# lbcb-sci/raven

Measured on AMD Instinct MI355X. Metric: read Gbase/s through overlap+polish, higher is better.
Workload: dtype u32

## Files before the change

### raven_amd/csrc/engine.h

```cpp
#pragma once

#include <atomic>
#include <memory>
#include <mutex>
#include <string>
#include <vector>

#include "common.h"

namespace rvn {

constexpr int kSketchTile = 1024;
constexpr int kMaxWindow = 256;

inline u64 next_reads_serial() {
  static std::atomic<u64> counter{0};
  return ++counter;
}

struct ReadsDev {
  u32 n = 0;
  u64 total_bases = 0;
  u64 n_words = 0;
  DevBuf packed;
// ... 23 lines not shown
};

struct Index {
  u64 m = 0;
  u64 u = 0;
  int table_bits = 0;
  int shift = 0;
  DevBuf s_val[2];
  DevBuf s_org[2];
  int cur = 0;
  DevBuf u_val;
  DevBuf u_start;
  DevBuf table;
  DevBuf direct;
  bool direct_built = false;
  u32 occurrence = 0xFFFFFFFFu;
  bool table_built = false;
  bool has_query_flags = false;
  bool all_query = false;
  u32 first = 0, last = 0;
};

struct MapOut {
  u32 first = 0, last = 0;
  u64 n_query = 0;
  u64 n_matches = 0;
  u64 n_intervals = 0;
  u64 n_overlaps = 0;
  DevBuf ovl;
  DevBuf ovl_read_off;
// ... 8 lines not shown
  enum { kSketch, kSort, kIndex, kFilter, kQuery, kMatch, kSegSort, kIntervals, kChain, kCompact, kMerge, kPile,
         kTruncate, kNum };
  double ms[kNum] = {};
  u64 launches[kNum] = {};
};

struct PileState;
struct PileRegion;
struct ResolveState;

struct EngineOptions {
  long long nw_budget_mb = 0;
  long long nw_group_walk = 0;
  long long nw_stripe_lanes = 0;
  long long index_direct_min_keys = 0;
  long long poa_rows_min_windows = -1;
  long long io_threads = 0;
  long long io_slab_mb = 0;
  long long io_ring = 0;
  long long io_zlib = 0;
  long long arena_mb = 0;
  long long arena_margin_mb = 0;
  long long no_arena = 0;
  long long release_always = 0;
  long long polish_join = 0;
  long long polish_sketch_cache_mb = -1;
};
const char* engine_option_names();
long long* engine_option(EngineOptions& o, const char* name);

// ... 15 lines not shown
  u64 shard_join_matches = 0;
  MapOut map_out;
  DevBuf tmp_a, tmp_b, tmp_c, tmp_d, tmp_e, tmp_f, scan_tmp, sort_tmp;
  DevBuf sh_hist, sh_off, sh_ptrs;
  DevBuf q_start, q_cnt, m_off;
  struct PolishSketch {
    u32 first = 0, last = 0;
    Sketch sk;
  };
  u64 polish_sketch_owner = 0;
  std::vector<std::unique_ptr<PolishSketch>> polish_sketches;
  DevBuf pl_tval, pl_torg;
  DevBuf foreign_val, foreign_org;
  DevBuf sketch_sum;
  DevBuf m_grp[2], m_pos[2];
  DevBuf seg_off, iv_slot_begin, iv_slot_end, iv_cnt, iv_off, iv_begin, iv_end;
  DevBuf lis_min, lis_pred, lis_tail, lis_mask, ovl_slots, ovl_flags, ovl_scan, chain_big;
  DevBuf poa_scratch, poa2_scratch, polish_quals;
  DevBuf ed_cnt, ed_sort, ed_todo;
  DevBuf p2_slot, p2_pairs, p2_dist, p2_regions, p2_index_of, p2_kmers_off, p2_ok, p2_keep, p2_tmp_ovl;
  DevBuf io_text[2];
  int stage_kind = 0;
  u32 oom_mask = 0;
  std::vector<std::pair<std::unique_ptr<PinBuf>, bool>> io_pin;
  DevBuf poa_sched, poa_redo_w, poa_redo_i;
  DevBuf nw_hs, nw_ck, nw_hs2, nw_ck2, nw_hs3, nw_ck3, nw_hs4, nw_ck4, nw_strip, nw_jobs, nw_res;
  double nw_rate = -1.0;
  DevBuf pl_best, pl_best_t, pl_idmap, pl_recs, pl_keep, pl_win_cnt, pl_win_off, pl_win_fill, pl_win_meta, pl_first_window,
      pl_keys, pl_lays_tmp, pl_lays, pl_wins, pl_out, pl_len, pl_status, pl_ok, pl_cons_off, pl_final, pl_qual_off, pl_misc;
  std::vector<u64> pl_last_off;
// ... 302 lines not shown
```

### raven_amd/csrc/engine.hip

```cpp
#include <chrono>
#include <memory>

#include "abi.h"
#include "poa.h"

using namespace rvn;

static_assert(sizeof(rvn_overlap) == sizeof(rvn::Overlap), "overlap layout");

namespace {

thread_local std::string g_err;

const char* kStageNames[StageTimes::kNum] = {"sketch", "sort", "index", "filter", "query_sketch", "match",
                                             "seg_sort", "intervals", "chain", "compact", "merge", "pile",
                                             "truncate"};

void swap_bufs(DevBuf& a, DevBuf& b) {
  std::swap(a.ptr, b.ptr);
  std::swap(a.cap, b.cap);
}

}

// ... 62 lines not shown
  }
}

void fetch_values(Engine& e, const DevBuf& val, u64 n, u64* values) {
  if (!values || n == 0) return;
  if (e.val64) {
    RVN_HIP(hipMemcpy(values, val.ptr, n * 8, hipMemcpyDeviceToHost));
  } else {
    std::vector<u32> tmp(n);
    RVN_HIP(hipMemcpy(tmp.data(), val.ptr, n * 4, hipMemcpyDeviceToHost));
    for (u64 i = 0; i < n; ++i) values[i] = tmp[i];
  }
}

const char* engine_option_names() {
  return "nw_budget_mb, nw_group_walk, nw_stripe_lanes, index_direct_min_keys, poa_rows_min_windows, io_threads, io_slab_mb, io_ring, io_zlib, arena_mb, arena_margin_mb, "
         "no_arena, release_always, polish_join, polish_sketch_cache_mb";
}
long long* engine_option(EngineOptions& o, const char* name) {
  const std::string n(name ? name : "");
  if (n == "nw_budget_mb") return &o.nw_budget_mb;
  if (n == "nw_group_walk") return &o.nw_group_walk;
  if (n == "nw_stripe_lanes") return &o.nw_stripe_lanes;
  if (n == "index_direct_min_keys") return &o.index_direct_min_keys;
  if (n == "poa_rows_min_windows") return &o.poa_rows_min_windows;
  if (n == "io_threads") return &o.io_threads;
  if (n == "io_slab_mb") return &o.io_slab_mb;
  if (n == "io_ring") return &o.io_ring;
  if (n == "io_zlib") return &o.io_zlib;
  if (n == "arena_mb") return &o.arena_mb;
  if (n == "arena_margin_mb") return &o.arena_margin_mb;
  if (n == "no_arena") return &o.no_arena;
  if (n == "release_always") return &o.release_always;
  if (n == "polish_join") return &o.polish_join;
  if (n == "polish_sketch_cache_mb") return &o.polish_sketch_cache_mb;
  return nullptr;
}

void engine_release_scratch(Engine& e) {
  if (e.stream) (void)rvn_stream_sync(e.stream);
  e.query_ready = false;
  DevBuf* bufs[] = {
      &e.index.s_val[0], &e.index.s_val[1], &e.index.s_org[0], &e.index.s_org[1], &e.index.u_val, &e.index.u_start,
      &e.index.table, &e.index.direct, &e.index_sketch.val, &e.index_sketch.org, &e.index_sketch.read_off, &e.query_sketch.val,
      &e.query_sketch.org, &e.query_sketch.read_off, &e.raw_sketch.val, &e.raw_sketch.org, &e.raw_sketch.read_off,
      &e.map_out.ovl, &e.map_out.ovl_read_off, &e.map_out.filtered, &e.map_out.anchors, &e.map_out.anchor_off,
      &e.map_out.anchor_cnt, &e.tmp_a, &e.tmp_b, &e.tmp_c, &e.tmp_d, &e.tmp_e, &e.tmp_f, &e.scan_tmp, &e.sort_tmp,
      &e.q_start, &e.q_cnt, &e.m_off, &e.m_grp[0], &e.m_grp[1], &e.m_pos[0], &e.m_pos[1], &e.seg_off, &e.iv_slot_begin,
      &e.iv_slot_end, &e.iv_cnt, &e.iv_off, &e.iv_begin, &e.iv_end, &e.lis_min, &e.lis_pred, &e.lis_tail, &e.lis_mask,
      &e.ovl_slots, &e.ovl_flags, &e.ovl_scan, &e.chain_big, &e.sh_hist, &e.sh_off, &e.sh_ptrs, &e.poa_scratch, &e.poa2_scratch, &e.polish_quals, &e.ed_cnt, &e.ed_sort, &e.ed_todo, &e.p2_slot,
      &e.p2_pairs, &e.p2_dist, &e.p2_regions, &e.p2_index_of, &e.p2_kmers_off, &e.p2_ok, &e.p2_keep, &e.p2_tmp_ovl,
      &e.poa_sched, &e.poa_redo_w, &e.poa_redo_i, &e.nw_hs, &e.nw_ck, &e.nw_hs2, &e.nw_ck2, &e.nw_hs3, &e.nw_ck3, &e.nw_hs4, &e.nw_ck4, &e.nw_strip, &e.nw_jobs, &e.nw_res,
      &e.pl_best, &e.pl_best_t, &e.pl_idmap, &e.pl_recs, &e.pl_keep, &e.pl_win_cnt, &e.pl_win_off, &e.pl_win_fill,
      &e.pl_win_meta, &e.pl_first_window, &e.pl_keys, &e.pl_lays_tmp, &e.pl_lays, &e.pl_wins, &e.pl_out, &e.pl_len,
      &e.pl_status, &e.pl_ok, &e.pl_cons_off, &e.pl_final, &e.pl_qual_off, &e.pl_misc, &e.anc_slot_off, &e.anc_slot_cnt};
  for (DevBuf* b : bufs) b->release();
  e.pl_last_valid = false;
  e.polish_sketches.clear();
  e.polish_sketch_owner = 0;
  e.pl_tval.release();
  e.pl_torg.release();
  e.foreign_val.release();
  e.foreign_org.release();
  e.index.m = e.index.u = 0;
  e.index.table_built = false;
  e.index.direct_built = false;
  e.map_out.n_query = e.map_out.n_matches = e.map_out.n_intervals = e.map_out.n_overlaps = 0;
  e.map_out.first = e.map_out.last = 0;
  e.map_out.has_anchors = false;
  e.polish_last_windows = 0;
  e.polish_last_layers = 0;
  delete e.pile_pool;
  e.pile_pool = nullptr;
}
void engine_release_scratch_if_tight(Engine& e, int stage_kind) {
  e.stage_kind = stage_kind;
  size_t free_b = 0, total_b = 0;
  if (hipMemGetInfo(&free_b, &total_b) != hipSuccess) return;
  const bool trace = knob("RVN_DEBUG_MEM") != nullptr;
  if (devpool::active()) {
    const size_t afree = devpool::free_total(), asize = devpool::size();
// ... 188 lines not shown
```

### raven_amd/csrc/index.hip

```cpp
#include <algorithm>
#include <vector>

#include "engine.h"
#include "wave.h"

namespace rvn {

namespace {

template <typename V>
__global__ void heads_kernel(const V* __restrict__ val, u64 n, u8* __restrict__ flags) {
  u64 i = static_cast<u64>(blockIdx.x) * blockDim.x + threadIdx.x;
  if (i < n) flags[i] = (i == 0 || val[i] != val[i - 1]) ? 1 : 0;
}

template <typename V>
__global__ void unique_kernel(const V* __restrict__ val, const u8* __restrict__ flags, const u32* __restrict__ scan,
                              u64 n, V* __restrict__ u_val, u32* __restrict__ u_start, u32 u) {
  u64 i = static_cast<u64>(blockIdx.x) * blockDim.x + threadIdx.x;
  if (i < n && flags[i]) {
    u32 j = scan[i];
    u_val[j] = val[i];
    u_start[j] = static_cast<u32>(i);
  }
// ... 23 lines not shown
    for (u32 i = lane; i < n; i += 64) table[s + i] = v;
  }
}

template <typename V>
__global__ __launch_bounds__(256) void table_tail_kernel(const V* __restrict__ u_val, u32 u, int shift, u32 B,
                                                        u32* __restrict__ table) {
  const u64 first = (static_cast<u64>(u_val[u - 1]) >> shift) + 1;
  for (u64 b = first + static_cast<u64>(blockIdx.x) * blockDim.x + threadIdx.x; b <= B;
       b += static_cast<u64>(gridDim.x) * blockDim.x)
    table[b] = u;
}

template <typename V>
__global__ __launch_bounds__(256) void direct_fill_kernel(const V* __restrict__ u_val, const u32* __restrict__ u_start, u32 u,
                                                         u64* __restrict__ direct) {
  const u32 j = blockIdx.x * 256 + threadIdx.x;
  if (j >= u) return;
  const u32 a = u_start[j], b = u_start[j + 1];
  direct[static_cast<u64>(u_val[j])] = (static_cast<u64>(b - a) << 32) | a;
}

__global__ void table_empty_kernel(u32* table, u32 B) {
  u32 i = blockIdx.x * blockDim.x + threadIdx.x;
  if (i <= B) table[i] = 0;
}

constexpr u32 kHistBins = 65536;

__global__ __launch_bounds__(256) void occ_hist_kernel(const u32* __restrict__ u_start, u32 u,
                                                      u32* __restrict__ hist, u32* __restrict__ overflow_list,
                                                      u32* __restrict__ overflow_n, u32 overflow_cap,
                                                      const u64* __restrict__ s_org) {
  __shared__ u32 lh[256];
  lh[threadIdx.x] = 0;
// ... 52 lines not shown
  StageTimer t(e, StageTimes::kIndex);
  const V* sv = ix.s_val[ix.cur].as<V>();
  u8* flags = e.tmp_c.get<u8>(m + 1);
  u32* fscan = e.tmp_d.get<u32>(m + 1);
  RVN_KLAUNCH(kKHeads, heads_kernel<V><<<div_up(m, 256), 256, 0, s>>>(sv, m, flags));
  exclusive_scan_u8_u32(flags, fscan, m, e.scan_tmp, s);
  const u32 u = static_cast<u32>(read_back(e, fscan + m, 4));
  ix.u = u;
  V* u_val = ix.u_val.get<V>(static_cast<size_t>(u) + 1);
  u32* u_start = ix.u_start.get<u32>(static_cast<size_t>(u) + 2);
  RVN_KLAUNCH(kKUnique, unique_kernel<V><<<div_up(m, 256), 256, 0, s>>>(sv, flags, fscan, m, u_val, u_start, u));
  t.stop();
}

constexpr u32 kDirectMinKeys = 8u << 20;

template <typename V>
void index_table_impl(Engine& e) {
  hipStream_t s = e.stream;
  Index& ix = e.index;
  if (ix.table_built || ix.m == 0) return;
  StageTimer t(e, StageTimes::kIndex);
  const u32 u = static_cast<u32>(ix.u);
  int bits = 1;
  while ((1ULL << bits) < 2ULL * u) ++bits;
  bits = std::max(8, bits);
  bits = std::min(bits, std::min<int>(2 * e.k, 26));
  ix.table_bits = bits;
  ix.shift = 2 * e.k - bits;
  const u32 B = 1u << bits;
  u32* table = ix.table.get<u32>(static_cast<size_t>(B) + 2);
  const V* u_val = ix.u_val.as<V>();
  RVN_KLAUNCH(kKTable, table_kernel<V><<<div_up(u, 256), 256, 0, s>>>(u_val, u, ix.shift, table);
              table_tail_kernel<V><<<256, 256, 0, s>>>(u_val, u, ix.shift, B, table));
  ix.table_built = true;
  ix.direct_built = false;
  const u64 direct_min = e.opt.index_direct_min_keys > 0 ? static_cast<u64>(e.opt.index_direct_min_keys) : kDirectMinKeys;
  if (sizeof(V) == 4 && 2 * e.k <= 30 && u >= direct_min && !knob("RVN_NO_DIRECT_INDEX")) {
    const size_t n_dir = static_cast<size_t>(1) << (2 * e.k);
    u64* direct = nullptr;
    try {
      direct = ix.direct.get<u64>(n_dir);
    } catch (const DeviceOutOfMemory&) {
      direct = nullptr;
    }
    if (direct) {
      RVN_HIP(hipMemsetAsync(direct, 0, n_dir * 8, s));
      RVN_KLAUNCH(kKTable, direct_fill_kernel<V><<<div_up(u, 256), 256, 0, s>>>(u_val, ix.u_start.as<u32>(), u, direct));
      ix.direct_built = true;
    }
  }
  t.stop();
}

template <typename V>
void index_build_impl(Engine& e, Sketch& sk, bool build_table) {
  hipStream_t s = e.stream;
  Index& ix = e.index;
  const u64 m = sk.count;
  ix.m = m;
  ix.u = 0;
  ix.occurrence = 0xFFFFFFFFu;
  if (m >= (1ULL << 32)) throw HipError("[raven_hip] index batch with >= 2^32 minimizers is not supported");

  std::swap(ix.s_val[0].ptr, sk.val.ptr);
  std::swap(ix.s_val[0].cap, sk.val.cap);
  std::swap(ix.s_org[0].ptr, sk.org.ptr);
  std::swap(ix.s_org[0].cap, sk.org.cap);
  ix.cur = 0;
  if (m == 0) {
    ix.table_bits = 1;
    ix.shift = 2 * e.k > 1 ? 2 * e.k - 1 : 0;
    u32* table = ix.table.get<u32>(3);
    RVN_KLAUNCH(kKTable, table_empty_kernel<<<1, 64, 0, s>>>(table, 2));
    ix.u_val.reserve(16);
    ix.u_start.reserve(16);
    RVN_HIP(hipMemsetAsync(ix.u_start.ptr, 0, 8, s));
    ix.table_built = true;
    ix.direct_built = false;
    return;
  }
  V* v0 = ix.s_val[0].as<V>();
  u64* o0 = ix.s_org[0].as<u64>();
  V* v1 = ix.s_val[1].get<V>(m + 1);
  u64* o1 = ix.s_org[1].get<u64>(m + 1);
  {
    StageTimer t(e, StageTimes::kSort);
    if (sizeof(V) == 4)
      ix.cur = radix_sort_pairs_u32_u64(reinterpret_cast<u32*>(v0), reinterpret_cast<u32*>(v1), o0, o1, m, 2 * e.k,
                                        e.sort_tmp, e.scan_tmp, s, kKRsUpsweep, kKRsDownsweep, false);
    else
      ix.cur = radix_sort_pairs_u64_u64(reinterpret_cast<u64*>(v0), reinterpret_cast<u64*>(v1), o0, o1, m, 2 * e.k,
                                        e.sort_tmp, e.scan_tmp, s, kKRsUpsweep, kKRsDownsweep, false);
    t.stop();
  }
  ix.table_built = false;
  ix.direct_built = false;
  index_runs_impl<V>(e);
  if (build_table) index_table_impl<V>(e);
}

}

void index_build(Engine& e, Sketch& sk, bool build_table) {
  e.index.first = sk.first;
  e.index.last = sk.last;
  if (e.val64) index_build_impl<u64>(e, sk, build_table);
  else index_build_impl<u32>(e, sk, build_table);
}

void index_build_table(Engine& e) {
  if (e.val64) index_table_impl<u64>(e);
// ... 66 lines not shown
```

### raven_amd/csrc/map.hip

```cpp
#include <algorithm>

#include <cstring>

#include "engine.h"
#include "wave.h"

namespace rvn {

namespace {

template <typename V>
__device__ __forceinline__ bool index_find(const V* __restrict__ u_val, const u32* __restrict__ u_start,
                                           const u32* __restrict__ table, int shift, V v, u32* start, u32* count) {
  const u32 b = static_cast<u32>(static_cast<u64>(v) >> shift);
  u32 lo = table[b], hi = table[b + 1];
  const u32 end = hi;
  while (lo < hi) {
    const u32 mid = lo + ((hi - lo) >> 1);
    if (u_val[mid] < v) lo = mid + 1;
    else hi = mid;
  }
  if (lo < end && u_val[lo] == v) {
    *start = u_start[lo];
    *count = u_start[lo + 1] - *start;
    return true;
  }
  return false;
}

template <typename V>
__global__ void match_count_kernel(const V* __restrict__ q_val, const u64* __restrict__ q_org, u64 nq,
                                   const V* __restrict__ u_val, const u32* __restrict__ u_start,
                                   const u32* __restrict__ table, int shift, u32 n_keys,
                                   const u64* __restrict__ s_org, u32 occurrence, int avoid_equal,
                                   int avoid_symmetric, u32* __restrict__ q_start, u32* __restrict__ q_n,
                                   u32* __restrict__ q_cnt, u8* __restrict__ filtered, const u64* __restrict__ direct) {
  u64 q = static_cast<u64>(blockIdx.x) * blockDim.x + threadIdx.x;
  if (q >= nq) return;
  const V v = q_val[q];
  const u32 qid = origin_id(q_org[q]);
  u32 start = 0, count = 0, cnt = 0;
  u8 filt = 0;
  bool found;
  if (direct) {
    const u64 ent = direct[static_cast<u64>(v)];
    count = static_cast<u32>(ent >> 32);
    found = count != 0;
    start = found ? static_cast<u32>(ent) : 0u;
  } else {
    found = n_keys && index_find<V>(u_val, u_start, table, shift, v, &start, &count);
  }
  if (found) {
    if (count > occurrence) {
      filt = 1;
      count = 0;
    } else {
      for (u32 j = 0; j < count; ++j) {
        const u32 rid = origin_id(s_org[start + j]);
        if (avoid_equal && qid == rid) continue;
        if (avoid_symmetric && qid > rid) continue;
        ++cnt;
      }
    }
  }
  q_start[q] = start;
  q_n[q] = count;
  q_cnt[q] = cnt;
  if (filtered) filtered[q] = filt;
}

__global__ void match_emit_kernel(const u64* __restrict__ q_org, u64 nq, const u64* __restrict__ s_org,
                                  const u32* __restrict__ q_start, const u32* __restrict__ q_n,
                                  const u64* __restrict__ m_off, int avoid_equal, int avoid_symmetric,
                                  u64* __restrict__ m_grp, u64* __restrict__ m_pos) {
  u64 q = static_cast<u64>(blockIdx.x) * blockDim.x + threadIdx.x;
  if (q >= nq) return;
  const u32 count = q_n[q];
  if (count == 0) return;
  const u64 qo = q_org[q];
  const u32 qid = origin_id(qo);
  const u64 lhs_pos = static_cast<u32>(qo) >> 1;
  const u32 qstrand = static_cast<u32>(qo) & 1u;
  const u32 start = q_start[q];
  u64 o = m_off[q];
  for (u32 j = 0; j < count; ++j) {
    const u64 ro = s_org[start + j];
    const u32 rid = origin_id(ro);
    if (avoid_equal && qid == rid) continue;
    if (avoid_symmetric && qid > rid) continue;
    const u64 rhs_pos = static_cast<u32>(ro) >> 1;
    const u64 strand = (qstrand == (static_cast<u32>(ro) & 1u)) ? 1 : 0;
    const u64 diagonal = !strand ? rhs_pos + lhs_pos : rhs_pos - lhs_pos + (3ULL << 30);
    m_grp[o] = (((static_cast<u64>(rid) << 1) | strand) << 32) | diagonal;
    m_pos[o] = (lhs_pos << 32) | rhs_pos;
    ++o;
  }
}

template <bool EMIT>
__global__ __launch_bounds__(256) void join_kernel(const u32* __restrict__ u_start, u32 n_runs,
                                                  const u64* __restrict__ s_org, u32 occurrence, int all_query,
                                                  int avoid_equal, int avoid_symmetric, u32 first, u32 q_lo, u32 q_hi,
                                                  u32* __restrict__ read_cnt, const u64* __restrict__ seg_off,
                                                  u32* __restrict__ cursor, u64* __restrict__ m_grp,
                                                  u64* __restrict__ m_pos) {
  const u32 run = blockIdx.x * blockDim.x + threadIdx.x;
  if (run >= n_runs) return;
  const u32 s = u_start[run];
  const u32 c = u_start[run + 1] - s;
  const u32 f = run_foreign_prefix(s_org, s, c);
// ... 135 lines not shown
  }
  if (cur) {
    for (u64 i = lane; i < n; i += 64) {
      k0[b + i] = k1[b + i];
      if (PAY) p0[b + i] = p1[b + i];
    }
    __threadfence_block();
  }
}

template <int NT, bool PAY>
constexpr size_t seg_sort_lds_bytes(u32 cap) {
  return static_cast<size_t>(cap) * 8 * (PAY ? 4 : 2) + (NT / 64) * 256 * 2 + 32 + (NT / 64) * 16;
}
template <int NT, bool PAY>
__device__ void block_sort_lds(u64* __restrict__ keys, u64* __restrict__ pays, u64 b, u32 n, u32 cap, unsigned char* smem) {
  constexpr int NW = NT / 64;
  static_assert(NT == 64 || NT == 256, "one wave or four");
  u64* s_k = reinterpret_cast<u64*>(smem);
  u64* s_p = s_k + 2 * static_cast<size_t>(cap);
  u16* wave_cnt = reinterpret_cast<u16*>(s_p + (PAY ? 2 * static_cast<size_t>(cap) : 0));
  u32* s4 = reinterpret_cast<u32*>(wave_cnt + NW * 256);
  u64* s_or = reinterpret_cast<u64*>(s4 + 8);
  u64* s_and = s_or + NW;
  const int lane = lane_id();
  const int w = threadIdx.x >> 6;
  u64 o = 0, a = ~0ULL;
  for (u32 i = threadIdx.x; i < n; i += NT) {
    const u64 k = keys[b + i];
    s_k[i] = k;
    if (PAY) s_p[i] = pays[b + i];
    o |= k;
    a &= k;
  }
#pragma unroll
  for (int x = 32; x > 0; x >>= 1) {
    o |= __shfl_xor(o, x, 64);
    a &= __shfl_xor(a, x, 64);
  }
  if (lane == 0) {
    s_or[w] = o;
    s_and[w] = a;
  }
  __syncthreads();
  u64 all_or = 0, all_and = ~0ULL;
#pragma unroll
// ... 73 lines not shown
    }
    __syncthreads();
    cur ^= 1;
  }
  const u64* kfin = s_k + static_cast<size_t>(cur) * cap;
  const u64* pfin = s_p + static_cast<size_t>(cur) * cap;
  for (u32 i = threadIdx.x; i < n; i += NT) {
    keys[b + i] = kfin[i];
    if (PAY) pays[b + i] = pfin[i];
  }
}

constexpr int kSegClasses = 5;
__constant__ u32 kSegClassCap[kSegClasses] = {256, 512, 1024, 2048, 4096};
static const u32 kSegClassCapHost[kSegClasses] = {256, 512, 1024, 2048, 4096};
__global__ __launch_bounds__(256) void seg_class_list_kernel(const u64* __restrict__ off, u32 n_seg, u32* __restrict__ lists,
                                                            u32* __restrict__ cnt) {
  const u32 t = blockIdx.x * blockDim.x + threadIdx.x;
  int cls = -1;
  if (t < n_seg) {
    const u64 n = off[t + 1] - off[t];
    if (n >= 2) {
      cls = kSegClasses;
      for (int c = kSegClasses - 1; c >= 0; --c)
        if (n <= kSegClassCap[c]) cls = c;
    }
  }
  const int lane = lane_id();
  for (int c = 0; c <= kSegClasses; ++c) {
    const unsigned long long m = __ballot(cls == c);
    if (!m) continue;
    u32 base = 0;
    if (lane == 0) base = atomicAdd(cnt + c, static_cast<u32>(__popcll(m)));
    base = __shfl(base, 0, 64);
    if (cls == c) lists[static_cast<size_t>(c) * n_seg + base + __popcll(m & ((1ULL << lane) - 1ULL))] = t;
  }
}
template <int NT>
__global__ __launch_bounds__(NT) void seg_sort_group_lds_kernel(u64* __restrict__ keys, u64* __restrict__ pays,
                                                               const u64* __restrict__ off, const u32* __restrict__ list,
                                                               u32 n_list, u32 cap) {
  extern __shared__ __attribute__((aligned(16))) unsigned char seg_smem[];
  if (blockIdx.x >= n_list) return;
  const u32 seg = list[blockIdx.x];
  const u64 b = off[seg];
  block_sort_lds<NT, true>(keys, pays, b, static_cast<u32>(off[seg + 1] - b), cap, seg_smem);
}
__global__ __launch_bounds__(256) void seg_sort_group_big_kernel(u64* k0, u64* k1, u64* p0, u64* p1, const u64* __restrict__ off,
                                                                const u32* __restrict__ list, u32 n_list) {
  __shared__ u32 hist[4][512];
  const u32 q = blockIdx.x * 4 + (threadIdx.x >> 6);
  if (q >= n_list) return;
  const u32 seg = list[q];
  const u64 b = off[seg], e = off[seg + 1];
  wave_sort_segment<true>(k0, k1, p0, p1, b, e - b, hist[threadIdx.x >> 6]);
}

template <int NT>
__global__ __launch_bounds__(NT) void seg_sort_pos_lds_kernel(u64* __restrict__ pos, const u64* __restrict__ iv_begin,
                                                             const u64* __restrict__ iv_end, const u32* __restrict__ list,
                                                             u32 n_list, u32 cap) {
  extern __shared__ __attribute__((aligned(16))) unsigned char seg_smem[];
  if (blockIdx.x >= n_list) return;
  const u32 t = list[blockIdx.x];
  const u64 b = iv_begin[t];
  block_sort_lds<NT, false>(pos, nullptr, b, static_cast<u32>(iv_end[t] - b), cap, seg_smem);
}
__global__ __launch_bounds__(256) void seg_sort_pos_big_kernel(u64* k0, u64* k1, const u64* __restrict__ iv_begin,
                                                              const u64* __restrict__ iv_end, const u32* __restrict__ list,
                                                              u32 n_list) {
  __shared__ u32 hist[4][512];
  const u32 q = blockIdx.x * 4 + (threadIdx.x >> 6);
  if (q >= n_list) return;
  const u32 t = list[q];
  const u64 b = iv_begin[t], e = iv_end[t];
  wave_sort_segment<false>(k0, k1, nullptr, nullptr, b, e - b, hist[threadIdx.x >> 6]);
}

__global__ __launch_bounds__(256) void intervals_kernel(const u64* __restrict__ grp, const u64* __restrict__ seg_off,
                                                       u32 n_seg, u64 bandwidth, u64* __restrict__ slot_begin,
                                                       u64* __restrict__ slot_end, u32* __restrict__ iv_cnt) {
// ... 524 lines not shown
                                   const u8* __restrict__ flags, const u32* __restrict__ scan, u64 n_slots,
                                   u64* __restrict__ aoff, u32* __restrict__ acnt) {
  u64 i = static_cast<u64>(blockIdx.x) * blockDim.x + threadIdx.x;
  if (i < n_slots && flags[i]) {
    aoff[scan[i]] = slot_aoff[i];
    acnt[scan[i]] = slot_acnt[i];
  }
}

__global__ void read_ovl_off_kernel(const u64* __restrict__ seg_off, const u32* __restrict__ scan, u32 slot_div,
                                    u32 n, u32* __restrict__ out) {
  u32 i = blockIdx.x * blockDim.x + threadIdx.x;
  if (i < n) out[i] = scan[(seg_off[i] + slot_div - 1) / slot_div];
}

}

void chain_matches(Engine& e, const ReadsDev& r, u32 first, u32 last, u64 H, MapOut& out) {
  hipStream_t s = e.stream;
  const u32 nr = last - first;
  u32* ovl_read_off = out.ovl_read_off.get<u32>(static_cast<size_t>(nr) + 1);
  u64* seg_off = e.seg_off.as<u64>();
  if (H == 0) {
    RVN_HIP(hipMemsetAsync(ovl_read_off, 0, (static_cast<size_t>(nr) + 1) * 4, s));
    return;
  }
  u64* g0 = e.m_grp[0].as<u64>();
  u64* g1 = e.m_grp[1].as<u64>();
  u64* p0 = e.m_pos[0].as<u64>();
  u64* p1 = e.m_pos[1].as<u64>();
  {
    StageTimer t(e, StageTimes::kSegSort);
    u32* lists = e.chain_big.get<u32>(static_cast<size_t>(nr) * (kSegClasses + 1) + 16);
    u32* d_cnt = lists + static_cast<size_t>(nr) * (kSegClasses + 1);
    RVN_HIP(hipMemsetAsync(d_cnt, 0, (kSegClasses + 1) * 4, s));
    seg_class_list_kernel<<<div_up(nr, 256), 256, 0, s>>>(seg_off, nr, lists, d_cnt);
    RVN_LAUNCH_CHECK();
    read_back(e, d_cnt, (kSegClasses + 1) * 4);
    u32 n_cls[kSegClasses + 1];
    std::memcpy(n_cls, e.h_pin, sizeof(n_cls));
    static bool attr_set = false;
    if (!attr_set) {
      RVN_HIP(hipFuncSetAttribute(reinterpret_cast<const void*>(seg_sort_group_lds_kernel<256>),
                                  hipFuncAttributeMaxDynamicSharedMemorySize,
                                  static_cast<int>(seg_sort_lds_bytes<256, true>(kSegClassCapHost[kSegClasses - 1]))));
      attr_set = true;
    }
    if (n_cls[kSegClasses])
      RVN_KLAUNCH(kKSegSortGroup, seg_sort_group_big_kernel<<<div_up(n_cls[kSegClasses], 4), 256, 0, s>>>(
                                      g0, g1, p0, p1, seg_off, lists + static_cast<size_t>(kSegClasses) * nr, n_cls[kSegClasses]));
    for (int c = kSegClasses - 1; c >= 0; --c) {
      if (!n_cls[c]) continue;
      const u32 cap = kSegClassCapHost[c];
      const u32* list = lists + static_cast<size_t>(c) * nr;
      if (cap <= 512)
        RVN_KLAUNCH(kKSegSortGroup, seg_sort_group_lds_kernel<64><<<n_cls[c], 64, seg_sort_lds_bytes<64, true>(cap), s>>>(
                                        g0, p0, seg_off, list, n_cls[c], cap));
      else
        RVN_KLAUNCH(kKSegSortGroup, seg_sort_group_lds_kernel<256><<<n_cls[c], 256, seg_sort_lds_bytes<256, true>(cap), s>>>(
                                        g0, p0, seg_off, list, n_cls[c], cap));
    }
    t.stop();
  }
  u32 NI = 0;
  const u64 n_slots4 = (H + 3) / 4 + 1;
// ... 177 lines not shown
  if (nq == 0 || ix.m == 0) {
    RVN_HIP(hipMemsetAsync(ovl_read_off, 0, (static_cast<size_t>(nr) + 1) * 4, s));
    if (want_filtered) {
      u8* f = out.filtered.get<u8>(nq + 1);
      RVN_HIP(hipMemsetAsync(f, 0, nq + 1, s));
    }
    return;
  }
  {
    StageTimer t(e, StageTimes::kMatch);
    u32* q_start = e.q_start.get<u32>(nq + 1);
    u32* q_n = e.tmp_a.get<u32>(nq + 1);
    u32* q_cnt = e.q_cnt.get<u32>(nq + 1);
    u8* filt = want_filtered ? out.filtered.get<u8>(nq + 1) : nullptr;
    u64* m_off = e.m_off.get<u64>(nq + 2);
    RVN_KLAUNCH(kKMatchCount, match_count_kernel<V><<<div_up(nq, 256), 256, 0, s>>>(
        qs.val.as<V>(), qs.org.as<u64>(), nq, ix.u_val.as<V>(), ix.u_start.as<u32>(), ix.table.as<u32>(), ix.shift,
        static_cast<u32>(ix.u), ix.s_org[ix.cur].as<u64>(), ix.occurrence, avoid_equal, avoid_symmetric, q_start, q_n,
        q_cnt, filt, ix.direct_built ? ix.direct.as<u64>() : nullptr));
    exclusive_scan_u32_u64(q_cnt, m_off, nq, e.scan_tmp, s);
    H = read_back(e, m_off + nq, 8);
    out.n_matches = H;
    e.c_matches += H;
    if (H) {
      u64* g0 = e.m_grp[0].get<u64>(H + 1);
      u64* p0 = e.m_pos[0].get<u64>(H + 1);
      e.m_grp[1].reserve((H + 1) * 8);
      e.m_pos[1].reserve((H + 1) * 8);
      RVN_KLAUNCH(kKMatchEmit, match_emit_kernel<<<div_up(nq, 256), 256, 0, s>>>(qs.org.as<u64>(), nq, ix.s_org[ix.cur].as<u64>(), q_start,
                                                        q_n, m_off, avoid_equal, avoid_symmetric, g0, p0));
    }
    if (H) {
      RVN_KLAUNCH(kKGather, gather_u64_by_u32_kernel<<<div_up(nr + 1, 256), 256, 0, s>>>(
                                e.m_off.as<u64>(), qs.read_off.as<u32>(), seg_off, nr + 1));
// ... 92 lines not shown
```

Baseline: 1.418.

## Split big segment sorts via radix partitioning, wave-balanced match emit, presence bitmap

```diff
diff --git a/raven_amd/csrc/engine.h b/raven_amd/csrc/engine.h
--- a/raven_amd/csrc/engine.h
+++ b/raven_amd/csrc/engine.h
@@ -61,6 +61,8 @@
   DevBuf table;
   DevBuf direct;
   bool direct_built = false;
+  DevBuf present;
+  bool present_built = false;
   u32 occurrence = 0xFFFFFFFFu;
   bool table_built = false;
   bool has_query_flags = false;
@@ -99,6 +101,8 @@
   long long nw_group_walk = 0;
   long long nw_stripe_lanes = 0;
   long long index_direct_min_keys = 0;
+  long long index_presence_bits = 0;
+  long long seg_split_cap = 0;
   long long poa_rows_min_windows = -1;
   long long io_threads = 0;
   long long io_slab_mb = 0;
@@ -144,6 +148,7 @@
   DevBuf foreign_val, foreign_org;
   DevBuf sketch_sum;
   DevBuf m_grp[2], m_pos[2];
+  DevBuf seg_part;
   DevBuf seg_off, iv_slot_begin, iv_slot_end, iv_cnt, iv_off, iv_begin, iv_end;
   DevBuf lis_min, lis_pred, lis_tail, lis_mask, ovl_slots, ovl_flags, ovl_scan, chain_big;
   DevBuf poa_scratch, poa2_scratch, polish_quals;
diff --git a/raven_amd/csrc/engine.hip b/raven_amd/csrc/engine.hip
--- a/raven_amd/csrc/engine.hip
+++ b/raven_amd/csrc/engine.hip
@@ -100,7 +100,7 @@
 }
 
 const char* engine_option_names() {
-  return "nw_budget_mb, nw_group_walk, nw_stripe_lanes, index_direct_min_keys, poa_rows_min_windows, io_threads, io_slab_mb, io_ring, io_zlib, arena_mb, arena_margin_mb, "
+  return "nw_budget_mb, nw_group_walk, nw_stripe_lanes, index_direct_min_keys, index_presence_bits, seg_split_cap, poa_rows_min_windows, io_threads, io_slab_mb, io_ring, io_zlib, arena_mb, arena_margin_mb, "
          "no_arena, release_always, polish_join, polish_sketch_cache_mb";
 }
 long long* engine_option(EngineOptions& o, const char* name) {
@@ -109,6 +109,8 @@
   if (n == "nw_group_walk") return &o.nw_group_walk;
   if (n == "nw_stripe_lanes") return &o.nw_stripe_lanes;
   if (n == "index_direct_min_keys") return &o.index_direct_min_keys;
+  if (n == "index_presence_bits") return &o.index_presence_bits;
+  if (n == "seg_split_cap") return &o.seg_split_cap;
   if (n == "poa_rows_min_windows") return &o.poa_rows_min_windows;
   if (n == "io_threads") return &o.io_threads;
   if (n == "io_slab_mb") return &o.io_slab_mb;
@@ -128,7 +130,7 @@
   e.query_ready = false;
   DevBuf* bufs[] = {
       &e.index.s_val[0], &e.index.s_val[1], &e.index.s_org[0], &e.index.s_org[1], &e.index.u_val, &e.index.u_start,
-      &e.index.table, &e.index.direct, &e.index_sketch.val, &e.index_sketch.org, &e.index_sketch.read_off, &e.query_sketch.val,
+      &e.index.table, &e.index.direct, &e.index.present, &e.seg_part, &e.index_sketch.val, &e.index_sketch.org, &e.index_sketch.read_off, &e.query_sketch.val,
       &e.query_sketch.org, &e.query_sketch.read_off, &e.raw_sketch.val, &e.raw_sketch.org, &e.raw_sketch.read_off,
       &e.map_out.ovl, &e.map_out.ovl_read_off, &e.map_out.filtered, &e.map_out.anchors, &e.map_out.anchor_off,
       &e.map_out.anchor_cnt, &e.tmp_a, &e.tmp_b, &e.tmp_c, &e.tmp_d, &e.tmp_e, &e.tmp_f, &e.scan_tmp, &e.sort_tmp,
@@ -151,6 +153,7 @@
   e.index.m = e.index.u = 0;
   e.index.table_built = false;
   e.index.direct_built = false;
+  e.index.present_built = false;
   e.map_out.n_query = e.map_out.n_matches = e.map_out.n_intervals = e.map_out.n_overlaps = 0;
   e.map_out.first = e.map_out.last = 0;
   e.map_out.has_anchors = false;
diff --git a/raven_amd/csrc/index.hip b/raven_amd/csrc/index.hip
--- a/raven_amd/csrc/index.hip
+++ b/raven_amd/csrc/index.hip
@@ -61,11 +61,13 @@
 
 template <typename V>
 __global__ __launch_bounds__(256) void direct_fill_kernel(const V* __restrict__ u_val, const u32* __restrict__ u_start, u32 u,
-                                                         u64* __restrict__ direct) {
+                                                         u64* __restrict__ direct, u32* __restrict__ present) {
   const u32 j = blockIdx.x * 256 + threadIdx.x;
   if (j >= u) return;
   const u32 a = u_start[j], b = u_start[j + 1];
-  direct[static_cast<u64>(u_val[j])] = (static_cast<u64>(b - a) << 32) | a;
+  const u64 v = static_cast<u64>(u_val[j]);
+  direct[v] = (static_cast<u64>(b - a) << 32) | a;
+  if (present) atomicOr(present + (v >> 5), 1u << (v & 31));
 }
 
 __global__ void table_empty_kernel(u32* table, u32 B) {
@@ -148,6 +150,7 @@
 }
 
 constexpr u32 kDirectMinKeys = 8u << 20;
+constexpr bool kPresenceBitsDefault = false;
 
 template <typename V>
 void index_table_impl(Engine& e) {
@@ -169,6 +172,7 @@
               table_tail_kernel<V><<<256, 256, 0, s>>>(u_val, u, ix.shift, B, table));
   ix.table_built = true;
   ix.direct_built = false;
+  ix.present_built = false;
   const u64 direct_min = e.opt.index_direct_min_keys > 0 ? static_cast<u64>(e.opt.index_direct_min_keys) : kDirectMinKeys;
   if (sizeof(V) == 4 && 2 * e.k <= 30 && u >= direct_min && !knob("RVN_NO_DIRECT_INDEX")) {
     const size_t n_dir = static_cast<size_t>(1) << (2 * e.k);
@@ -179,9 +183,21 @@
       direct = nullptr;
     }
     if (direct) {
+      u32* present = nullptr;
+      const bool want_bits = e.opt.index_presence_bits == 1 || (e.opt.index_presence_bits != 2 && kPresenceBitsDefault);
+      const size_t n_words = std::max<size_t>(1, n_dir >> 5);
+      if (want_bits) {
+        try {
+          present = ix.present.get<u32>(n_words);
+        } catch (const DeviceOutOfMemory&) {
+          present = nullptr;
+        }
+      }
       RVN_HIP(hipMemsetAsync(direct, 0, n_dir * 8, s));
-      RVN_KLAUNCH(kKTable, direct_fill_kernel<V><<<div_up(u, 256), 256, 0, s>>>(u_val, ix.u_start.as<u32>(), u, direct));
+      if (present) RVN_HIP(hipMemsetAsync(present, 0, n_words * 4, s));
+      RVN_KLAUNCH(kKTable, direct_fill_kernel<V><<<div_up(u, 256), 256, 0, s>>>(u_val, ix.u_start.as<u32>(), u, direct, present));
       ix.direct_built = true;
+      ix.present_built = present != nullptr;
     }
   }
   t.stop();
@@ -212,6 +228,7 @@
     RVN_HIP(hipMemsetAsync(ix.u_start.ptr, 0, 8, s));
     ix.table_built = true;
     ix.direct_built = false;
+    ix.present_built = false;
     return;
   }
   V* v0 = ix.s_val[0].as<V>();
@@ -230,6 +247,7 @@
   }
   ix.table_built = false;
   ix.direct_built = false;
+  ix.present_built = false;
   index_runs_impl<V>(e);
   if (build_table) index_table_impl<V>(e);
 }
diff --git a/raven_amd/csrc/map.hip b/raven_amd/csrc/map.hip
--- a/raven_amd/csrc/map.hip
+++ b/raven_amd/csrc/map.hip
@@ -28,22 +28,23 @@
   return false;
 }
 
-template <typename V>
+template <typename V, bool WALK>
 __global__ void match_count_kernel(const V* __restrict__ q_val, const u64* __restrict__ q_org, u64 nq,
                                    const V* __restrict__ u_val, const u32* __restrict__ u_start,
                                    const u32* __restrict__ table, int shift, u32 n_keys,
                                    const u64* __restrict__ s_org, u32 occurrence, int avoid_equal,
                                    int avoid_symmetric, u32* __restrict__ q_start, u32* __restrict__ q_n,
-                                   u32* __restrict__ q_cnt, u8* __restrict__ filtered, const u64* __restrict__ direct) {
+                                   u32* __restrict__ q_cnt, u8* __restrict__ filtered, const u64* __restrict__ direct,
+                                   const u32* __restrict__ present) {
   u64 q = static_cast<u64>(blockIdx.x) * blockDim.x + threadIdx.x;
   if (q >= nq) return;
   const V v = q_val[q];
-  const u32 qid = origin_id(q_org[q]);
   u32 start = 0, count = 0, cnt = 0;
   u8 filt = 0;
   bool found;
   if (direct) {
-    const u64 ent = direct[static_cast<u64>(v)];
+    u64 ent = 0;
+    if (!present || ((present[static_cast<u64>(v) >> 5] >> (static_cast<u32>(v) & 31)) & 1u)) ent = direct[static_cast<u64>(v)];
     count = static_cast<u32>(ent >> 32);
     found = count != 0;
     start = found ? static_cast<u32>(ent) : 0u;
@@ -54,13 +55,16 @@
     if (count > occurrence) {
       filt = 1;
       count = 0;
-    } else {
+    } else if (WALK) {
+      const u32 qid = origin_id(q_org[q]);
       for (u32 j = 0; j < count; ++j) {
         const u32 rid = origin_id(s_org[start + j]);
         if (avoid_equal && qid == rid) continue;
         if (avoid_symmetric && qid > rid) continue;
         ++cnt;
       }
+    } else {
+      cnt = count;
     }
   }
   q_start[q] = start;
@@ -69,31 +73,58 @@
   if (filtered) filtered[q] = filt;
 }
 
-__global__ void match_emit_kernel(const u64* __restrict__ q_org, u64 nq, const u64* __restrict__ s_org,
-                                  const u32* __restrict__ q_start, const u32* __restrict__ q_n,
-                                  const u64* __restrict__ m_off, int avoid_equal, int avoid_symmetric,
-                                  u64* __restrict__ m_grp, u64* __restrict__ m_pos) {
-  u64 q = static_cast<u64>(blockIdx.x) * blockDim.x + threadIdx.x;
-  if (q >= nq) return;
-  const u32 count = q_n[q];
-  if (count == 0) return;
-  const u64 qo = q_org[q];
-  const u32 qid = origin_id(qo);
-  const u64 lhs_pos = static_cast<u32>(qo) >> 1;
-  const u32 qstrand = static_cast<u32>(qo) & 1u;
-  const u32 start = q_start[q];
-  u64 o = m_off[q];
-  for (u32 j = 0; j < count; ++j) {
-    const u64 ro = s_org[start + j];
-    const u32 rid = origin_id(ro);
-    if (avoid_equal && qid == rid) continue;
-    if (avoid_symmetric && qid > rid) continue;
-    const u64 rhs_pos = static_cast<u32>(ro) >> 1;
-    const u64 strand = (qstrand == (static_cast<u32>(ro) & 1u)) ? 1 : 0;
-    const u64 diagonal = !strand ? rhs_pos + lhs_pos : rhs_pos - lhs_pos + (3ULL << 30);
-    m_grp[o] = (((static_cast<u64>(rid) << 1) | strand) << 32) | diagonal;
-    m_pos[o] = (lhs_pos << 32) | rhs_pos;
-    ++o;
+__global__ __launch_bounds__(256) void match_emit_kernel(const u64* __restrict__ q_org, u64 nq, const u64* __restrict__ s_org,
+                                                        const u32* __restrict__ q_start, const u32* __restrict__ q_n,
+                                                        const u64* __restrict__ m_off, int avoid_equal, int avoid_symmetric,
+                                                        u64* __restrict__ m_grp, u64* __restrict__ m_pos) {
+  __shared__ u32 s_incl[4][64];
+  const int lane = lane_id();
+  u32* incl = s_incl[threadIdx.x >> 6];
+  const u64 q = static_cast<u64>(blockIdx.x) * blockDim.x + threadIdx.x;
+  if (q - lane >= nq) return;
+  const bool in = q < nq;
+  const u32 count = in ? q_n[q] : 0u;
+  const u32 my_incl = wave_inclusive_sum(count);
+  const u32 total = __shfl(my_incl, 63, 64);
+  if (total == 0) return;
+  const u64 my_org = in ? q_org[q] : 0ULL;
+  const u32 my_start = in ? q_start[q] : 0u;
+  const u32 my_excl = my_incl - count;
+  u64 o = in && lane == 0 ? m_off[q] : 0ULL;
+  o = __shfl(o, 0, 64);
+  incl[lane] = my_incl;
+  __builtin_amdgcn_wave_barrier();
+  const unsigned long long lt = lanemask_lt();
+  for (u32 base = 0; base < total; base += 64) {
+    const u32 c = base + static_cast<u32>(lane);
+    const bool valid = c < total;
+    int src = 0;
+#pragma unroll
+    for (int step = 32; step > 0; step >>= 1)
+      if (incl[src + step - 1] <= c) src += step;
+    if (!valid) src = 63;
+    const u64 qo = __shfl(my_org, src, 64);
+    const u32 start = __shfl(my_start, src, 64);
+    const u32 j = c - __shfl(my_excl, src, 64);
+    bool keep = false;
+    u64 ro = 0;
+    if (valid) {
+      ro = s_org[start + j];
+      const u32 qid = origin_id(qo), rid = origin_id(ro);
+      keep = !(avoid_equal && qid == rid) && !(avoid_symmetric && qid > rid);
+    }
+    const unsigned long long kept = __ballot(keep);
+    if (keep) {
+      const u64 lhs_pos = static_cast<u32>(qo) >> 1;
+      const u32 qstrand = static_cast<u32>(qo) & 1u;
+      const u64 rhs_pos = static_cast<u32>(ro) >> 1;
+      const u64 strand = (qstrand == (static_cast<u32>(ro) & 1u)) ? 1 : 0;
+      const u64 diagonal = !strand ? rhs_pos + lhs_pos : rhs_pos - lhs_pos + (3ULL << 30);
+      const u64 at = o + __popcll(kept & lt);
+      m_grp[at] = (((static_cast<u64>(origin_id(ro)) << 1) | strand) << 32) | diagonal;
+      m_pos[at] = (lhs_pos << 32) | rhs_pos;
+    }
+    o += __popcll(kept);
   }
 }
 
@@ -259,7 +290,8 @@
   return static_cast<size_t>(cap) * 8 * (PAY ? 4 : 2) + (NT / 64) * 256 * 2 + 32 + (NT / 64) * 16;
 }
 template <int NT, bool PAY>
-__device__ void block_sort_lds(u64* __restrict__ keys, u64* __restrict__ pays, u64 b, u32 n, u32 cap, unsigned char* smem) {
+__device__ void block_sort_lds(const u64* ksrc, const u64* psrc, u64* keys, u64* pays, u64 b, u32 n, u32 cap,
+                               unsigned char* smem) {
   constexpr int NW = NT / 64;
   static_assert(NT == 64 || NT == 256, "one wave or four");
   u64* s_k = reinterpret_cast<u64*>(smem);
@@ -272,9 +304,9 @@
   const int w = threadIdx.x >> 6;
   u64 o = 0, a = ~0ULL;
   for (u32 i = threadIdx.x; i < n; i += NT) {
-    const u64 k = keys[b + i];
+    const u64 k = ksrc[b + i];
     s_k[i] = k;
-    if (PAY) s_p[i] = pays[b + i];
+    if (PAY) s_p[i] = psrc[b + i];
     o |= k;
     a &= k;
   }
@@ -378,16 +410,17 @@
 constexpr int kSegClasses = 5;
 __constant__ u32 kSegClassCap[kSegClasses] = {256, 512, 1024, 2048, 4096};
 static const u32 kSegClassCapHost[kSegClasses] = {256, 512, 1024, 2048, 4096};
-__global__ __launch_bounds__(256) void seg_class_list_kernel(const u64* __restrict__ off, u32 n_seg, u32* __restrict__ lists,
-                                                            u32* __restrict__ cnt) {
+__global__ __launch_bounds__(256) void seg_class_list_kernel(const u64* __restrict__ off, u32 n_seg, u32 split_cap,
+                                                            u32* __restrict__ lists, u32* __restrict__ cnt) {
   const u32 t = blockIdx.x * blockDim.x + threadIdx.x;
   int cls = -1;
   if (t < n_seg) {
     const u64 n = off[t + 1] - off[t];
     if (n >= 2) {
       cls = kSegClasses;
-      for (int c = kSegClasses - 1; c >= 0; --c)
-        if (n <= kSegClassCap[c]) cls = c;
+      if (n <= split_cap)
+        for (int c = kSegClasses - 1; c >= 0; --c)
+          if (n <= kSegClassCap[c]) cls = c;
     }
   }
   const int lane = lane_id();
@@ -408,16 +441,189 @@
   if (blockIdx.x >= n_list) return;
   const u32 seg = list[blockIdx.x];
   const u64 b = off[seg];
-  block_sort_lds<NT, true>(keys, pays, b, static_cast<u32>(off[seg + 1] - b), cap, seg_smem);
-}
-__global__ __launch_bounds__(256) void seg_sort_group_big_kernel(u64* k0, u64* k1, u64* p0, u64* p1, const u64* __restrict__ off,
-                                                                const u32* __restrict__ list, u32 n_list) {
-  __shared__ u32 hist[4][512];
-  const u32 q = blockIdx.x * 4 + (threadIdx.x >> 6);
-  if (q >= n_list) return;
-  const u32 seg = list[q];
-  const u64 b = off[seg], e = off[seg + 1];
-  wave_sort_segment<true>(k0, k1, p0, p1, b, e - b, hist[threadIdx.x >> 6]);
+  block_sort_lds<NT, true>(keys, pays, keys, pays, b, static_cast<u32>(off[seg + 1] - b), cap, seg_smem);
+}
+struct PartItem {
+  u64 b;
+  u32 n;
+  u32 tile_base;
+};
+struct PartLevel {
+  PartItem* items;
+  u64* bits;
+  u32* tile_item;
+  u32* cnt;
+};
+__device__ __forceinline__ void part_item_emit(const PartLevel& lv, u64 b, u32 n, u32 tile) {
+  const u32 nt = (n + tile - 1) / tile;
+  const u32 idx = atomicAdd(lv.cnt, 1u);
+  const u32 tb = atomicAdd(lv.cnt + 1, nt);
+  lv.items[idx] = PartItem{b, n, tb};
+  lv.bits[2 * idx] = 0;
+  lv.bits[2 * idx + 1] = ~0ULL;
+  for (u32 t = 0; t < nt; ++t) lv.tile_item[tb + t] = idx;
+}
+__device__ __forceinline__ int part_shift(u64 o, u64 a) {
+  const u64 varying = o ^ a;
+  if (!varying) return 0;
+  const int top = 63 - __clzll(static_cast<long long>(varying));
+  return top > 7 ? top - 7 : 0;
+}
+__global__ __launch_bounds__(256) void seg_part_init_kernel(const u64* __restrict__ off, const u32* __restrict__ list,
+                                                           u32 n_list, u32 tile, PartLevel lv) {
+  const u32 t = blockIdx.x * blockDim.x + threadIdx.x;
+  if (t >= n_list) return;
+  const u32 seg = list[t];
+  part_item_emit(lv, off[seg], static_cast<u32>(off[seg + 1] - off[seg]), tile);
+}
+__global__ __launch_bounds__(256) void seg_part_bits_kernel(const u64* __restrict__ keys, u32 tile, PartLevel lv) {
+  const u32 it = lv.tile_item[blockIdx.x];
+  const PartItem item = lv.items[it];
+  const u32 lo = (blockIdx.x - item.tile_base) * tile, hi = min(item.n, lo + tile);
+  u64 o = 0, a = ~0ULL;
+  for (u32 i = lo + threadIdx.x; i < hi; i += 256) {
+    const u64 k = keys[item.b + i];
+    o |= k;
+    a &= k;
+  }
+#pragma unroll
+  for (int x = 32; x > 0; x >>= 1) {
+    o |= __shfl_xor(o, x, 64);
+    a &= __shfl_xor(a, x, 64);
+  }
+  if (lane_id() == 0) {
+    atomicOr(reinterpret_cast<unsigned long long*>(lv.bits + 2 * it), static_cast<unsigned long long>(o));
+    atomicAnd(reinterpret_cast<unsigned long long*>(lv.bits + 2 * it + 1), static_cast<unsigned long long>(a));
+  }
+}
+__global__ __launch_bounds__(256) void seg_part_hist_kernel(const u64* __restrict__ keys, u32 tile, PartLevel lv,
+                                                           u32* __restrict__ tile_hist) {
+  __shared__ u32 h[256];
+  const u32 it = lv.tile_item[blockIdx.x];
+  const PartItem item = lv.items[it];
+  const int shift = part_shift(lv.bits[2 * it], lv.bits[2 * it + 1]);
+  const u32 lo = (blockIdx.x - item.tile_base) * tile, hi = min(item.n, lo + tile);
+  h[threadIdx.x] = 0;
+  __syncthreads();
+  for (u32 i = lo + threadIdx.x; i < hi; i += 256) atomicAdd(&h[(keys[item.b + i] >> shift) & 0xFF], 1u);
+  __syncthreads();
+  tile_hist[static_cast<size_t>(blockIdx.x) * 256 + threadIdx.x] = h[threadIdx.x];
+}
+__global__ __launch_bounds__(256) void seg_part_plan_kernel(PartLevel lv, u32* __restrict__ tile_hist, u32 tile, u32 split_cap,
+                                                           int dst_is_side0, PartLevel next, u64* __restrict__ range_b,
+                                                           u32* __restrict__ range_n, u32* __restrict__ n_ranges) {
+  __shared__ u32 s4[4];
+  __shared__ u32 s_tot[256], s_start[256];
+  const u32 it = blockIdx.x;
+  const PartItem item = lv.items[it];
+  const int shift = part_shift(lv.bits[2 * it], lv.bits[2 * it + 1]);
+  const u32 nt = (item.n + tile - 1) / tile;
+  const u32 d = threadIdx.x;
+  u32 run = 0;
+  for (u32 t = 0; t < nt; ++t) {
+    u32* p = tile_hist + static_cast<size_t>(item.tile_base + t) * 256 + d;
+    const u32 c = *p;
+    *p = run;
+    run += c;
+  }
+  u32 total;
+  const u32 start = block_exclusive_sum_256<u32>(run, s4, &total);
+  for (u32 t = 0; t < nt; ++t) tile_hist[static_cast<size_t>(item.tile_base + t) * 256 + d] += start;
+  s_tot[d] = run;
+  s_start[d] = start;
+  __syncthreads();
+  if (d != 0) return;
+  auto range = [&](u32 at, u32 n) {
+    if (n == 0 || (n == 1 && dst_is_side0)) return;
+    const u32 r = atomicAdd(n_ranges, 1u);
+    range_b[r] = item.b + at;
+    range_n[r] = n;
+  };
+  u32 gb = 0, gn = 0;
+  for (u32 x = 0; x < 256; ++x) {
+    const u32 c = s_tot[x];
+    if (c == 0) continue;
+    if (c > split_cap) {
+      range(gb, gn);
+      gn = 0;
+      if (shift > 0) {
+        part_item_emit(next, item.b + s_start[x], c, tile);
+      } else if (!dst_is_side0) {
+        for (u32 at = 0; at < c; at += split_cap) range(s_start[x] + at, min(split_cap, c - at));
+      }
+    } else if (gn == 0 || gn + c > split_cap) {
+      range(gb, gn);
+      gb = s_start[x];
+      gn = c;
+    } else {
+      gn += c;
+    }
+  }
+  range(gb, gn);
+}
+__global__ __launch_bounds__(256) void seg_part_scatter_kernel(const u64* __restrict__ kin, const u64* __restrict__ pin,
+                                                              u64* __restrict__ kout, u64* __restrict__ pout, u32 tile,
+                                                              PartLevel lv, const u32* __restrict__ tile_hist) {
+  __shared__ u32 wave_at[4][256];
+  const u32 it = lv.tile_item[blockIdx.x];
+  const PartItem item = lv.items[it];
+  const int shift = part_shift(lv.bits[2 * it], lv.bits[2 * it + 1]);
+  const u32 lo = (blockIdx.x - item.tile_base) * tile, hi = min(item.n, lo + tile);
+  const int lane = lane_id();
+  const int w = threadIdx.x >> 6;
+  const unsigned long long lt = lanemask_lt();
+  const u32 per = tile / 4;
+  const u32 q0 = min(hi, lo + w * per), q1 = min(hi, q0 + per);
+  u32* my_at = wave_at[w];
+  for (int i = lane; i < 256; i += 64) my_at[i] = 0;
+  __builtin_amdgcn_wave_barrier();
+  for (u32 base = q0; base < q1; base += 64) {
+    const u32 i = base + lane;
+    const bool valid = i < q1;
+    const unsigned d = valid ? static_cast<unsigned>((kin[item.b + i] >> shift) & 0xFF) : 0;
+    const unsigned long long peers = match_digit8(d, valid);
+    if (valid && (peers & lt) == 0) my_at[d] += static_cast<u32>(__popcll(peers));
+    __builtin_amdgcn_wave_barrier();
+  }
+  __syncthreads();
+  {
+    u32 run = tile_hist[static_cast<size_t>(blockIdx.x) * 256 + threadIdx.x];
+#pragma unroll
+    for (int x = 0; x < 4; ++x) {
+      const u32 c = wave_at[x][threadIdx.x];
+      wave_at[x][threadIdx.x] = run;
+      run += c;
+    }
+  }
+  __syncthreads();
+  for (u32 base = q0; base < q1; base += 64) {
+    const u32 i = base + lane;
+    const bool valid = i < q1;
+    u64 k = 0, pv = 0;
+    if (valid) {
+      k = kin[item.b + i];
+      pv = pin[item.b + i];
+    }
+    const unsigned d = static_cast<unsigned>((k >> shift) & 0xFF);
+    const unsigned long long peers = match_digit8(d, valid);
+    u32 before = 0;
+    if (valid) before = my_at[d];
+    __builtin_amdgcn_wave_barrier();
+    if (valid && (peers & lt) == 0) my_at[d] = before + static_cast<u32>(__popcll(peers));
+    __builtin_amdgcn_wave_barrier();
+    if (valid) {
+      const u64 dst = item.b + before + __popcll(peers & lt);
+      kout[dst] = k;
+      pout[dst] = pv;
+    }
+  }
+}
+template <int NT>
+__global__ __launch_bounds__(NT) void seg_sort_group_range_kernel(const u64* ksrc, const u64* psrc, u64* keys, u64* pays,
+                                                                 const u64* __restrict__ range_b,
+                                                                 const u32* __restrict__ range_n, u32 cap) {
+  extern __shared__ __attribute__((aligned(16))) unsigned char seg_smem[];
+  block_sort_lds<NT, true>(ksrc, psrc, keys, pays, range_b[blockIdx.x], range_n[blockIdx.x], cap, seg_smem);
 }
 
 template <int NT>
@@ -428,7 +634,7 @@
   if (blockIdx.x >= n_list) return;
   const u32 t = list[blockIdx.x];
   const u64 b = iv_begin[t];
-  block_sort_lds<NT, false>(pos, nullptr, b, static_cast<u32>(iv_end[t] - b), cap, seg_smem);
+  block_sort_lds<NT, false>(pos, nullptr, pos, nullptr, b, static_cast<u32>(iv_end[t] - b), cap, seg_smem);
 }
 __global__ __launch_bounds__(256) void seg_sort_pos_big_kernel(u64* k0, u64* k1, const u64* __restrict__ iv_begin,
                                                               const u64* __restrict__ iv_end, const u32* __restrict__ list,
@@ -983,6 +1189,72 @@
   if (i < n) out[i] = scan[(seg_off[i] + slot_div - 1) / slot_div];
 }
 
+void sort_big_segments(Engine& e, u64* g0, u64* g1, u64* p0, u64* p1, const u64* seg_off, const u32* list, u32 n_list, u64 H,
+                       u32 split_cap) {
+  hipStream_t s = e.stream;
+  const u32 tile = split_cap < 2048 ? 256 : 2048;
+  const size_t max_items = std::max<size_t>(n_list, H / split_cap + 1);
+  const size_t max_tiles = H / tile + max_items + 1;
+  const size_t max_ranges = 5 * (H / split_cap) + 2 * max_items + 16;
+  const size_t words = 2 * (max_items * 8 + max_tiles) + max_ranges * 3 + 16;
+  u32* base = e.seg_part.get<u32>(words + 64);
+  PartLevel lv[2];
+  u32* cnt = base;
+  u64* p64 = reinterpret_cast<u64*>(base + 16);
+  for (int x = 0; x < 2; ++x) {
+    lv[x].items = reinterpret_cast<PartItem*>(p64);
+    p64 += 2 * max_items;
+    lv[x].bits = p64;
+    p64 += 2 * max_items;
+    lv[x].cnt = cnt + 2 * x;
+  }
+  u64* range_b = p64;
+  p64 += max_ranges;
+  u32* p32 = reinterpret_cast<u32*>(p64);
+  u32* range_n = p32;
+  p32 += max_ranges;
+  for (int x = 0; x < 2; ++x) {
+    lv[x].tile_item = p32;
+    p32 += max_tiles;
+  }
+  RVN_HIP(hipMemsetAsync(cnt, 0, 8 * 4, s));
+  RVN_KLAUNCH(kKSegSortGroup, seg_part_init_kernel<<<div_up(n_list, 256), 256, 0, s>>>(seg_off, list, n_list, tile, lv[0]));
+  u32 h[8];
+  read_back(e, cnt, sizeof(h));
+  std::memcpy(h, e.h_pin, sizeof(h));
+  for (int level = 0;; ++level) {
+    const int cur = level & 1;
+    const u32 n_items = h[2 * cur], n_tiles = h[2 * cur + 1];
+    if (n_items == 0) break;
+    if (level >= 8) throw HipError("[raven_hip] group sort: a segment is still split after eight levels");
+    if (n_items > max_items || n_tiles > max_tiles) throw HipError("[raven_hip] group sort: partition tables too small");
+    const u64* kin = cur ? g1 : g0;
+    const u64* pin = cur ? p1 : p0;
+    u64* kout = cur ? g0 : g1;
+    u64* pout = cur ? p0 : p1;
+    u32* tile_hist = e.tmp_f.get<u32>(static_cast<size_t>(n_tiles) * 256);
+    RVN_HIP(hipMemsetAsync(lv[cur ^ 1].cnt, 0, 8, s));
+    RVN_HIP(hipMemsetAsync(cnt + 4, 0, 4, s));
+    RVN_KLAUNCH(kKSegSortGroup, seg_part_bits_kernel<<<n_tiles, 256, 0, s>>>(kin, tile, lv[cur]));
+    RVN_KLAUNCH(kKSegSortGroup, seg_part_hist_kernel<<<n_tiles, 256, 0, s>>>(kin, tile, lv[cur], tile_hist));
+    RVN_KLAUNCH(kKSegSortGroup, seg_part_plan_kernel<<<n_items, 256, 0, s>>>(lv[cur], tile_hist, tile, split_cap, cur, lv[cur ^ 1],
+                                                                             range_b, range_n, cnt + 4));
+    RVN_KLAUNCH(kKSegSortGroup, seg_part_scatter_kernel<<<n_tiles, 256, 0, s>>>(kin, pin, kout, pout, tile, lv[cur], tile_hist));
+    read_back(e, cnt, sizeof(h));
+    std::memcpy(h, e.h_pin, sizeof(h));
+    const u32 n_ranges = h[4];
+    if (n_ranges > max_ranges) throw HipError("[raven_hip] group sort: range table too small");
+    if (n_ranges) {
+      if (split_cap <= 512)
+        RVN_KLAUNCH(kKSegSortGroup, seg_sort_group_range_kernel<64><<<n_ranges, 64, seg_sort_lds_bytes<64, true>(split_cap), s>>>(
+                                        kout, pout, g0, p0, range_b, range_n, split_cap));
+      else
+        RVN_KLAUNCH(kKSegSortGroup, seg_sort_group_range_kernel<256><<<n_ranges, 256, seg_sort_lds_bytes<256, true>(split_cap), s>>>(
+                                        kout, pout, g0, p0, range_b, range_n, split_cap));
+    }
+  }
+}
+
 }
 
 void chain_matches(Engine& e, const ReadsDev& r, u32 first, u32 last, u64 H, MapOut& out) {
@@ -1003,7 +1275,10 @@
     u32* lists = e.chain_big.get<u32>(static_cast<size_t>(nr) * (kSegClasses + 1) + 16);
     u32* d_cnt = lists + static_cast<size_t>(nr) * (kSegClasses + 1);
     RVN_HIP(hipMemsetAsync(d_cnt, 0, (kSegClasses + 1) * 4, s));
-    seg_class_list_kernel<<<div_up(nr, 256), 256, 0, s>>>(seg_off, nr, lists, d_cnt);
+    const u32 cap_max = kSegClassCapHost[kSegClasses - 1];
+    const u32 split_cap = e.opt.seg_split_cap > 0 ? static_cast<u32>(std::min<long long>(cap_max, std::max<long long>(16, e.opt.seg_split_cap)))
+                                                  : cap_max;
+    seg_class_list_kernel<<<div_up(nr, 256), 256, 0, s>>>(seg_off, nr, split_cap, lists, d_cnt);
     RVN_LAUNCH_CHECK();
     read_back(e, d_cnt, (kSegClasses + 1) * 4);
     u32 n_cls[kSegClasses + 1];
@@ -1012,12 +1287,14 @@
     if (!attr_set) {
       RVN_HIP(hipFuncSetAttribute(reinterpret_cast<const void*>(seg_sort_group_lds_kernel<256>),
                                   hipFuncAttributeMaxDynamicSharedMemorySize,
-                                  static_cast<int>(seg_sort_lds_bytes<256, true>(kSegClassCapHost[kSegClasses - 1]))));
+                                  static_cast<int>(seg_sort_lds_bytes<256, true>(cap_max))));
+      RVN_HIP(hipFuncSetAttribute(reinterpret_cast<const void*>(seg_sort_group_range_kernel<256>),
+                                  hipFuncAttributeMaxDynamicSharedMemorySize,
+                                  static_cast<int>(seg_sort_lds_bytes<256, true>(cap_max))));
       attr_set = true;
     }
     if (n_cls[kSegClasses])
-      RVN_KLAUNCH(kKSegSortGroup, seg_sort_group_big_kernel<<<div_up(n_cls[kSegClasses], 4), 256, 0, s>>>(
-                                      g0, g1, p0, p1, seg_off, lists + static_cast<size_t>(kSegClasses) * nr, n_cls[kSegClasses]));
+      sort_big_segments(e, g0, g1, p0, p1, seg_off, lists + static_cast<size_t>(kSegClasses) * nr, n_cls[kSegClasses], H, split_cap);
     for (int c = kSegClasses - 1; c >= 0; --c) {
       if (!n_cls[c]) continue;
       const u32 cap = kSegClassCapHost[c];
@@ -1225,10 +1502,17 @@
     u32* q_cnt = e.q_cnt.get<u32>(nq + 1);
     u8* filt = want_filtered ? out.filtered.get<u8>(nq + 1) : nullptr;
     u64* m_off = e.m_off.get<u64>(nq + 2);
-    RVN_KLAUNCH(kKMatchCount, match_count_kernel<V><<<div_up(nq, 256), 256, 0, s>>>(
-        qs.val.as<V>(), qs.org.as<u64>(), nq, ix.u_val.as<V>(), ix.u_start.as<u32>(), ix.table.as<u32>(), ix.shift,
-        static_cast<u32>(ix.u), ix.s_org[ix.cur].as<u64>(), ix.occurrence, avoid_equal, avoid_symmetric, q_start, q_n,
-        q_cnt, filt, ix.direct_built ? ix.direct.as<u64>() : nullptr));
+    const u64* direct = ix.direct_built ? ix.direct.as<u64>() : nullptr;
+    const u32* present = ix.direct_built && ix.present_built ? ix.present.as<u32>() : nullptr;
+    if (avoid_equal || avoid_symmetric)
+      RVN_KLAUNCH(kKMatchCount, match_count_kernel<V, true><<<div_up(nq, 256), 256, 0, s>>>(
+          qs.val.as<V>(), qs.org.as<u64>(), nq, ix.u_val.as<V>(), ix.u_start.as<u32>(), ix.table.as<u32>(), ix.shift,
+          static_cast<u32>(ix.u), ix.s_org[ix.cur].as<u64>(), ix.occurrence, avoid_equal, avoid_symmetric, q_start, q_n,
+          q_cnt, filt, direct, present));
+    else
+      RVN_KLAUNCH(kKMatchCount, match_count_kernel<V, false><<<div_up(nq, 256), 256, 0, s>>>(
+          qs.val.as<V>(), qs.org.as<u64>(), nq, ix.u_val.as<V>(), ix.u_start.as<u32>(), ix.table.as<u32>(), ix.shift,
+          static_cast<u32>(ix.u), ix.s_org[ix.cur].as<u64>(), ix.occurrence, 0, 0, q_start, q_n, q_cnt, filt, direct, present));
     exclusive_scan_u32_u64(q_cnt, m_off, nq, e.scan_tmp, s);
     H = read_back(e, m_off + nq, 8);
     out.n_matches = H;
```

Result: no change. 1.429 (median of 2 runs) (+0.8%).
